# astaka-pe/SeMIGCN

Measured on AMD Instinct MI355X. Metric: GCN train iters/sec + edges-aggregated/sec, 1M-vert mesh, higher is better.
Workload: dtype bf16 storage / f32 accumulate; 1 GPU; SGCN train iteration (13 ChebConv K=3 + BN + LeakyReLU, fwd+loss+bwd, Adam every 5th) on a closed torus mesh 1000x1000: V=1000000 E=6000000 directed, grid vertex order, bf16 features; V=1000000, E=6000000, vertex_order=grid

## Files before the change

### include/semigcn.h

```cpp
#ifndef SEMIGCN_H
#define SEMIGCN_H

#include <stdint.h>

#ifdef __cplusplus
extern "C" {
#endif

#if defined(__GNUC__)
#define SG_API __attribute__((visibility("default")))
#else
#define SG_API
#endif

#define SG_ABI_VERSION 1

enum sg_status {
  SG_OK = 0,
  SG_ERR_INVALID = -1,
  SG_ERR_HIP = -2,
  SG_ERR_UNSUPPORTED = -3,
  SG_ERR_NO_DEVICE = -4
};

// ... 128 lines not shown
SG_API int sg_fill_emit(sg_fill* s, const float* vs, float* new_vs, int64_t* new_faces, uint8_t* filled_out, void* stream);

typedef struct sg_parts sg_parts;
SG_API int sg_parts_create(const int64_t* faces, int64_t F, int64_t V, int connectivity, void* stream, sg_parts** out);
SG_API int sg_parts_destroy(sg_parts* p);
SG_API int sg_parts_query(const sg_parts* p, int64_t* info);
SG_API int sg_parts_labels(const sg_parts* p, int64_t* face_label, int64_t* face_count, void* stream);
SG_API int sg_parts_select(sg_parts* p, const uint8_t* keep, void* stream, int64_t* n_vertices, int64_t* n_faces);
SG_API int sg_parts_emit(sg_parts* p, const float* vs, float* new_vs, int64_t* new_faces, int64_t* vertex_ids, int64_t* face_ids,
                         void* stream);

typedef struct sg_remesh sg_remesh;
SG_API int sg_remesh_create(const float* vs, int64_t V, const int64_t* faces, int64_t F, void* stream, sg_remesh** out);
SG_API int sg_remesh_destroy(sg_remesh* p);
SG_API int sg_remesh_query(const sg_remesh* p, int64_t* info);
SG_API int sg_remesh_split(sg_remesh* p, float thr2, int64_t max_rounds, void* stream, int64_t* counts, int64_t* n_rounds,
                           int64_t* n_long);
SG_API int sg_remesh_flip(sg_remesh* p, int64_t max_rounds, void* stream, int64_t* counts, int64_t* n_rounds, int64_t* deviation);
SG_API int sg_remesh_collapse(sg_remesh* p, float lo2, float thr2, int64_t max_rounds, void* stream, int64_t* counts,
                              int64_t* n_rounds, int64_t* n_short);
SG_API int sg_remesh_collapse_maps(const sg_remesh* p, int64_t* vertex_ids, int64_t* merged_into, void* stream);
SG_API int sg_remesh_export(const sg_remesh* p, float* vs, int64_t* faces, int64_t* parents, uint8_t* border, void* stream);
SG_API int sg_remesh_set_feature(sg_remesh* p, int enabled, double cos_t);
SG_API int sg_remesh_features(sg_remesh* p, void* stream, uint8_t* vclass, int64_t* crease_nbr, int64_t* n_crease);
SG_API int sg_remesh_crease_edges(const sg_remesh* p, int64_t* edges, void* stream);
SG_API int sg_crease_step(const float* in, float* out, const int64_t* crease_nbr, int64_t V, void* stream);

SG_API int sg_mesh_loss_finalize(const float* partial, int64_t nb, float n_v, float n_f, float w_pos, float k1, float* out,
                                 void* stream);
SG_API int64_t sg_mesh_loss_blocks(int64_t V, int64_t F);
SG_API int sg_mesh_loss_fwd(const float* pos, const int64_t* faces, const float* target_pos, const float* v_keep,
                            const float* target_fn, const float* f_keep, int64_t V, int64_t F, float* partial,
                            void* stream);
SG_API int sg_mesh_loss_bwd_det(const float* pos, const int64_t* faces, const float* target_pos, const float* v_keep,
                                const float* target_fn, const float* f_keep, const float* g, int64_t V, int64_t V_ext,
                                int64_t F, const sg_pool* incidence, float* corner_scratch, float* grad_pos, void* stream);
SG_API int sg_mesh_loss_bwd(const float* pos, const int64_t* faces, const float* target_pos, const float* v_keep,
                            const float* target_fn, const float* f_keep, const float* g, int64_t V, int64_t V_ext,
                            int64_t F, float* grad_pos, void* stream);

SG_API int64_t sg_bnf_blocks(int64_t F);
SG_API int64_t sg_bnf_scratch_bytes(int64_t F);
SG_API int sg_bnf_filter(const float* pos, const int64_t* faces, const int64_t* f2f, int64_t V, int64_t F, int loop,
                         float sigma_s, const float* start_fn, float* fn, float* n_filtered, float* loss_partial,
                         void* scratch, void* stream);
SG_API int sg_mesh_loss_cad_finalize(const float* partial, int64_t nb, float n_v, float n_f, float w_pos, float k1,
                                     const float* bnf_partial, int64_t nb_bnf, int64_t F, float k2, float* out, void* stream);
SG_API int sg_mesh_loss_cad_bwd_det(const float* pos, const int64_t* faces, const float* target_pos, const float* v_keep,
                                    const float* target_fn, const float* f_keep, const float* fn, const float* n_filtered,
                                    const float* g, int64_t V, int64_t V_ext, int64_t F, const sg_pool* incidence,
                                    float* corner_scratch, float* grad_pos, void* stream);

SG_API int sg_gemm_nt_takes_big_tile(int64_t M, int64_t N, int64_t K, int64_t lda, int64_t ldb, int64_t ldc);
SG_API int64_t sg_gemm_tile_rows(int64_t N);
SG_API int64_t sg_gemm_row_tiles(int64_t M, int64_t N);
SG_API int sg_gemm_nt(const void* A, int64_t lda, const void* B, int64_t ldb, const float* bias, void* C, int64_t ldc,
                      int64_t M, int64_t N, int64_t K, int dtype, float* moments, void* stream);
SG_API int64_t sg_gemm_tn_slabs(int64_t M, int64_t N, int64_t Kp);
SG_API int sg_gemm_tn_takes_big_tile(int64_t M, int64_t N, int64_t Kp, int64_t lda, int64_t ldb);
SG_API int sg_gemm_tn(const void* A, int64_t lda, const void* B, int64_t ldb, int64_t M, int64_t N, int64_t Kp, int dtype,
                      float* workspace, float* out, int64_t ldo, void* stream);
SG_API int sg_gemm_nt_f32_supported(int64_t M, int64_t N, int64_t K, int64_t lda, int64_t ldc);
SG_API int sg_gemm_nt_f32_pays(int64_t M, int64_t N, int64_t K);
SG_API int sg_gemm_nt_f32_variant(int64_t M);
SG_API int64_t sg_gemm_nt_f32_workspace(int64_t N, int64_t K);
SG_API int sg_gemm_nt_f32(const float* A, int64_t lda, const float* W, int64_t w_rs, int64_t w_cs, const float* bias, float* C,
                          int64_t ldc, int64_t M, int64_t N, int64_t K, void* workspace, int64_t workspace_bytes, void* stream);
SG_API int sg_gemm_tn_f32_supported(int64_t M, int64_t N, int64_t Kp, int64_t lda, int64_t ldb);
SG_API int64_t sg_gemm_tn_f32_workspace(int64_t M, int64_t N, int64_t Kp);
SG_API int sg_gemm_tn_f32(const float* A, int64_t lda, const float* B, int64_t ldb, int64_t M, int64_t N, int64_t Kp,
                          void* workspace, int64_t workspace_bytes, float* out, int64_t ldo, void* stream);
SG_API int sg_bn_stats_finalize_tiles(const float* partial, int64_t n_tiles, int64_t rows_per_tile, int64_t V, int64_t C,
                                      const float* gamma, const float* beta, float* running_mean, float* running_var,
                                      float momentum, float eps, float* out, int64_t* batches_tracked, void* stream);

SG_API int sg_input_bounds(const float* z1, int64_t V, float* partial_values, int64_t* partial_index, float* bounds, int64_t* arg,
                           void* stream);
SG_API int sg_input_prep_bwd_routed(const void* gX, int64_t ldg, const float* z1, const float* dm, const int64_t* rank,
                                    const float* bounds, const int64_t* arg, float* dz1, float* partial, float* d_bounds,
                                    int64_t V, int dtype, void* stream);
SG_API int64_t sg_input_prep_blocks(int64_t V);
SG_API int sg_input_prep(const float* z1, const float* dm, const int64_t* order, const float* lo, const float* hi, void* X,
                         int64_t ldx, int64_t V, int dtype, void* stream);
SG_API int sg_input_prep_bwd(const void* gX, int64_t ldg, const float* z1, const float* dm, const int64_t* rank,
                             const float* lo, const float* hi, float* dz1, float* partial, float* d_lo, float* d_hi, int64_t V,
                             int dtype, void* stream);

typedef struct sg_block {
  const sg_graph* graph;
  const sg_pool* pool;
  int32_t pool_mode;
  int32_t dtype;
  int32_t K;
  int32_t order;
  int32_t training;
  int32_t refresh_weights;
  int32_t need_dx;
  int32_t reserved_;
  int64_t V, V_out;
  int64_t Cin, Cout;
  float momentum, eps, slope;
  float reserved2_;
  const float* W[3];
  const float* bias;
  const float* gamma;
  const float* beta;
// ... 111 lines not shown
```

### semigcn_amd/capi.py

```python
from __future__ import annotations

import ctypes
import functools
from array import array as _array
import os
from ctypes import POINTER, byref, c_char_p, c_float, c_int, c_int32, c_int64, c_void_p
from typing import Optional

import torch

_LIB_NAME = "libsemigcn_hip.so"
_LIB_PATH = os.path.join(os.path.dirname(os.path.abspath(__file__)), _LIB_NAME)

SG_F32, SG_BF16 = 0, 1
_DTYPES = {torch.float32: SG_F32, torch.bfloat16: SG_BF16}


class SemigcnLibraryError(RuntimeError):
    """libsemigcn_hip.so is absent / unloadable, or a call into it failed."""


class sg_graph_info(ctypes.Structure):
    _fields_ = [("V_dst", c_int64), ("V_src", c_int64), ("nnz", c_int64),
                ("symmetric", c_int32), ("max_degree", c_int32)]
# ... 21 lines not shown


PHASE_CONV, PHASE_BN, PHASE_BWD_REDUCE, PHASE_BWD_A, PHASE_BWD_B = 1, 2, 4, 8, 16


class sg_part_step(ctypes.Structure):
    _fields_ = [("kind", c_int32), ("reserved_", c_int32), ("blocks", POINTER(sg_block)), ("n", c_int64),
                ("send", c_void_p), ("recv", c_void_p)]


STEP_BLOCKS, STEP_EXCHANGE, STEP_ALL_REDUCE, STEP_ALL_GATHER = 0, 1, 2, 3


class sg_trace_record(ctypes.Structure):
    _fields_ = [("kind", c_int32), ("dtype", c_int32), ("engine", c_int32), ("reserved_", c_int32),
                ("a", c_int64), ("b", c_int64), ("c", c_int64), ("ms", c_float), ("reserved2_", c_float)]


_SIGNATURES = {
    "sg_last_error": (c_char_p, []),
    "sg_abi_version": (c_int, []),
    "sg_device_count": (c_int, []),
    "sg_graph_create": (c_int, [c_void_p, c_int64, c_int64, c_void_p, POINTER(c_void_p)]),
    "sg_graph_create_rect": (c_int, [c_void_p, c_void_p, c_int64, c_int64, c_int64, c_void_p, c_void_p,
                                     POINTER(c_void_p)]),
    "sg_graph_create_rows": (c_int, [c_void_p, c_void_p, c_int64, c_int64, c_int64, c_void_p, c_void_p, c_void_p, c_void_p,
                                     POINTER(c_void_p)]),
    "sg_graph_destroy": (c_int, [c_void_p]),
    "sg_graph_query": (c_int, [c_void_p, POINTER(sg_graph_info)]),
    "sg_graph_is_reordered": (c_int, [c_void_p]),
    "sg_graph_export": (c_int, [c_void_p, c_void_p, c_void_p, c_void_p, c_void_p]),
    "sg_spmm": (c_int, [c_void_p, c_int, c_void_p, c_int64, c_void_p, c_int64, c_void_p, c_int64,
                        c_void_p, c_int64, c_int64, c_int, c_float, c_float, c_float, c_void_p]),
    "sg_graph_prepare": (c_int, [c_void_p, c_int64, c_int, c_void_p]),
    "sg_pool_create": (c_int, [c_void_p, c_void_p, c_int64, c_int64, c_int64, c_void_p, POINTER(c_void_p)]),
    "sg_pool_destroy": (c_int, [c_void_p]),
    "sg_pool_mean": (c_int, [c_void_p, c_void_p, c_int64, c_void_p, c_int64, c_int64, c_int, c_void_p]),
    "sg_pool_mean_bwd": (c_int, [c_void_p, c_void_p, c_int64, c_void_p, c_int64, c_int64, c_int, c_void_p]),
    "sg_unpool": (c_int, [c_void_p, c_void_p, c_int64, c_void_p, c_int64, c_int64, c_int, c_void_p]),
    "sg_unpool_bwd": (c_int, [c_void_p, c_void_p, c_int64, c_void_p, c_int64, c_int64, c_int, c_void_p]),
    "sg_tuning_set": (c_int, [c_int, c_int]),
    "sg_mesh_loss_blocks": (c_int64, [c_int64, c_int64]),
    "sg_mesh_loss_fwd": (c_int, [c_void_p] * 6 + [c_int64, c_int64, c_void_p, c_void_p]),
    "sg_mesh_loss_bwd": (c_int, [c_void_p] * 7 + [c_int64, c_int64, c_int64, c_void_p, c_void_p]),
    "sg_mesh_loss_bwd_det": (c_int, [c_void_p] * 7 + [c_int64, c_int64, c_int64, c_void_p, c_void_p, c_void_p, c_void_p]),
    "sg_col_blocks": (c_int64, [c_int64]),
    "sg_col_moments": (c_int, [c_void_p, c_int64, c_int64, c_int64, c_int, c_void_p, c_int64, c_void_p]),
    "sg_bn_merge": (c_int, [c_void_p, c_int64, c_int64, c_int64, c_void_p, c_void_p]),
    "sg_bn_stats_finalize": (c_int, [c_void_p, c_int64, c_int64, c_int64, c_void_p, c_void_p, c_void_p, c_void_p, c_float,
                                     c_float, c_void_p, c_void_p, c_void_p]),
    "sg_bn_stats_finalize_tiles": (c_int, [c_void_p, c_int64, c_int64, c_int64, c_int64, c_void_p, c_void_p, c_void_p,
                                           c_void_p, c_float, c_float, c_void_p, c_void_p, c_void_p]),
    "sg_gemm_nt_takes_big_tile": (c_int, [c_int64, c_int64, c_int64, c_int64, c_int64, c_int64]),
    "sg_gemm_tile_rows": (c_int64, [c_int64]),
    "sg_gemm_row_tiles": (c_int64, [c_int64, c_int64]),
    "sg_gemm_nt": (c_int, [c_void_p, c_int64, c_void_p, c_int64, c_void_p, c_void_p, c_int64, c_int64, c_int64, c_int64,
                           c_int, c_void_p, c_void_p]),
    "sg_gemm_nt_f32_supported": (c_int, [c_int64, c_int64, c_int64, c_int64, c_int64]),
    "sg_gemm_nt_f32_pays": (c_int, [c_int64, c_int64, c_int64]),
    "sg_gemm_nt_f32_variant": (c_int, [c_int64]),
    "sg_gemm_nt_f32_workspace": (c_int64, [c_int64, c_int64]),
    "sg_gemm_nt_f32": (c_int, [c_void_p, c_int64, c_void_p, c_int64, c_int64, c_void_p, c_void_p, c_int64, c_int64, c_int64,
                               c_int64, c_void_p, c_int64, c_void_p]),
    "sg_gemm_tn_f32_supported": (c_int, [c_int64, c_int64, c_int64, c_int64, c_int64]),
    "sg_gemm_tn_f32_workspace": (c_int64, [c_int64, c_int64, c_int64]),
    "sg_gemm_tn_f32": (c_int, [c_void_p, c_int64, c_void_p, c_int64, c_int64, c_int64, c_int64, c_void_p, c_int64, c_void_p,
                               c_int64, c_void_p]),
    "sg_gemm_tn_slabs": (c_int64, [c_int64, c_int64, c_int64]),
    "sg_gemm_tn_takes_big_tile": (c_int, [c_int64, c_int64, c_int64, c_int64, c_int64]),
    "sg_gemm_tn": (c_int, [c_void_p, c_int64, c_void_p, c_int64, c_int64, c_int64, c_int64, c_int, c_void_p, c_void_p, c_int64,
                           c_void_p]),
    "sg_thin_supported": (c_int, [c_int64, c_int64]),
    "sg_thin_tn_blocks": (c_int64, [c_int64]),
    "sg_thin_nt": (c_int, [c_void_p, c_int64, c_void_p, c_int64, c_void_p, c_void_p, c_int64, c_int64, c_int64, c_int64, c_int,
                           c_void_p]),
    "sg_thin_tn": (c_int, [c_void_p, c_int64, c_void_p, c_int64, c_int64, c_int64, c_int64, c_int, c_void_p, c_void_p, c_int64,
                           c_void_p]),
    "sg_bn_bwd_coeffs": (c_int, [c_void_p, c_int64, c_int64, ctypes.c_double, c_void_p, c_void_p, c_void_p, c_void_p,
                                 c_void_p, c_void_p, c_void_p]),
    "sg_bn_merge_tiles": (c_int, [c_void_p, c_int64, c_int64, c_int64, c_int64, c_void_p, c_void_p, c_void_p]),
    "sg_multi_add": (c_int, [c_int64, c_void_p, c_void_p, c_void_p, c_void_p, c_void_p, c_void_p]),
    "sg_input_bounds": (c_int, [c_void_p, c_int64, c_void_p, c_void_p, c_void_p, c_void_p, c_void_p]),
    "sg_input_prep_bwd_routed": (c_int, [c_void_p, c_int64, c_void_p, c_void_p, c_void_p, c_void_p, c_void_p, c_void_p, c_void_p,
                                         c_void_p, c_int64, c_int, c_void_p]),
    "sg_mesh_loss_finalize": (c_int, [c_void_p, c_int64, c_float, c_float, c_float, c_float, c_void_p, c_void_p]),
    "sg_bnf_blocks": (c_int64, [c_int64]),
    "sg_bnf_scratch_bytes": (c_int64, [c_int64]),
    "sg_bnf_filter": (c_int, [c_void_p, c_void_p, c_void_p, c_int64, c_int64, c_int, c_float] + [c_void_p] * 6),
    "sg_mesh_loss_cad_finalize": (c_int, [c_void_p, c_int64, c_float, c_float, c_float, c_float, c_void_p, c_int64, c_int64, c_float,
                                          c_void_p, c_void_p]),
    "sg_mesh_loss_cad_bwd_det": (c_int, [c_void_p] * 9 + [c_int64, c_int64, c_int64, c_void_p, c_void_p, c_void_p, c_void_p]),
    "sg_input_prep_blocks": (c_int64, [c_int64]),
    "sg_input_prep": (c_int, [c_void_p, c_void_p, c_void_p, c_void_p, c_void_p, c_void_p, c_int64, c_int64, c_int, c_void_p]),
    "sg_input_prep_bwd": (c_int, [c_void_p, c_int64, c_void_p, c_void_p, c_void_p, c_void_p, c_void_p, c_void_p, c_void_p,
                                  c_void_p, c_void_p, c_int64, c_int, c_void_p]),
    "sg_bn_finalize_ranks": (c_int, [c_void_p, c_int64, c_int64, c_void_p, c_void_p, c_void_p, c_void_p, c_float, c_float,
                                     c_void_p, c_void_p, c_void_p, c_void_p]),
    "sg_bn_finalize": (c_int, [c_void_p, ctypes.c_double, c_int64, c_void_p, c_void_p, c_void_p, c_void_p, c_float,
                               c_float, c_void_p, c_void_p]),
    "sg_scale_shift_act": (c_int, [c_void_p, c_int64, c_void_p, c_void_p, c_float, c_void_p, c_int64, c_int64,
                                   c_int64, c_int, c_void_p]),
    "sg_bn_act_bwd_reduce": (c_int, [c_void_p, c_int64, c_void_p, c_int64, c_void_p, c_void_p, c_void_p, c_void_p,
                                     c_float, c_void_p, c_int64, c_int64, c_int64, c_int, c_void_p]),
    "sg_bn_act_bwd_apply": (c_int, [c_void_p, c_int64, c_void_p, c_int64, c_void_p, c_void_p, c_void_p, c_void_p,
                                    c_void_p, c_void_p, c_void_p, c_float, c_void_p, c_int64, c_int64, c_int64, c_int,
                                    c_void_p]),
# ... 513 lines not shown


def bn_stats_finalize(partial: torch.Tensor, num_rows: int, gamma: torch.Tensor, beta: torch.Tensor,
                      running_mean: Optional[torch.Tensor], running_var: Optional[torch.Tensor], momentum: float,
                      eps: float, batches_tracked: Optional[torch.Tensor] = None) -> torch.Tensor:
    nb, _, C = partial.shape
    out = torch.empty((4, C), dtype=torch.float32, device=partial.device)
    for t, n in ((running_mean, "running_mean"), (running_var, "running_var")):
        if t is not None:
            _f32vec(t, C, n)
    with _on_device(partial.device):
        _check(load().sg_bn_stats_finalize(_ptr(partial), nb, int(num_rows), C, _ptr(_f32vec(gamma, C, "weight")),
                                           _ptr(_f32vec(beta, C, "bias")), _ptr(running_mean), _ptr(running_var),
                                           float(momentum), float(eps), _ptr(out), _counter(batches_tracked, partial),
                                           _stream(partial)), "sg_bn_stats_finalize")
    return out


def bn_stats_finalize_tiles(partial: torch.Tensor, rows_per_tile: int, num_rows: int, gamma: torch.Tensor,
                            beta: torch.Tensor, running_mean: Optional[torch.Tensor], running_var: Optional[torch.Tensor],
                            momentum: float, eps: float, batches_tracked: Optional[torch.Tensor] = None) -> torch.Tensor:
    nb, _, C = partial.shape
    out = torch.empty((4, C), dtype=torch.float32, device=partial.device)
    for t, n in ((running_mean, "running_mean"), (running_var, "running_var")):
        if t is not None:
            _f32vec(t, C, n)
    with _on_device(partial.device):
        _check(load().sg_bn_stats_finalize_tiles(_ptr(partial), nb, int(rows_per_tile), int(num_rows), C,
                                                 _ptr(_f32vec(gamma, C, "weight")), _ptr(_f32vec(beta, C, "bias")),
                                                 _ptr(running_mean), _ptr(running_var), float(momentum), float(eps),
                                                 _ptr(out), _counter(batches_tracked, partial), _stream(partial)),
               "sg_bn_stats_finalize_tiles")
    return out


def gemm_tile_rows(N: int) -> int:
    return _sizes("sg_gemm_tile_rows", int(N))


def gemm_nt_supported(A: torch.Tensor, B: torch.Tensor, ldc: int) -> bool:
    if A.dtype != torch.bfloat16 or B.dtype != torch.bfloat16 or not A.is_cuda or A.dim() != 2 or B.dim() != 2:
        return False
    if A.shape[1] != B.shape[1] or A.stride(1) != 1 or B.stride(1) != 1 or A.shape[0] == 0:
        return False
    K, N = A.shape[1], B.shape[0]
    return (K % 8 == 0 and N % 8 == 0 and A.stride(0) % 8 == 0 and B.stride(0) % 8 == 0 and ldc % 8 == 0
            and A.data_ptr() % 16 == 0 and B.data_ptr() % 16 == 0)


def gemm_nt_takes_big_tile(M: int, N: int, K: int, lda: int, ldb: int, ldc: int) -> bool:
    return bool(_sizes("sg_gemm_nt_takes_big_tile", int(M), int(N), int(K), int(lda), int(ldb), int(ldc)))


def gemm_nt(A: torch.Tensor, B: torch.Tensor, bias: Optional[torch.Tensor] = None, out: Optional[torch.Tensor] = None,
            moments: bool = False):
    _require_device(A, "A")
    _require_device(B, "B")
    M, K = A.shape
    N = B.shape[0]
    if out is None:
        out = torch.empty((M, N), dtype=torch.bfloat16, device=A.device)
    if out.shape != (M, N) or out.dtype != torch.bfloat16 or B.shape[1] != K:
        raise SemigcnLibraryError(f"gemm_nt shape mismatch: A {tuple(A.shape)} B {tuple(B.shape)} out {tuple(out.shape)}")
    if bias is not None:
        _f32vec(bias, N, "bias")
    mom = None
    if moments:
        mom = torch.empty((_sizes("sg_gemm_row_tiles", M, N), 2, N), dtype=torch.float32, device=A.device)
    with _on_device(A.device):
        _check(load().sg_gemm_nt(_ptr(A), _rows2d(A, "A"), _ptr(B), _rows2d(B, "B"), _ptr(bias), _ptr(out),
                                 _rows2d(out, "out"), M, N, K, SG_BF16, _ptr(mom), _stream(A)), "sg_gemm_nt")
    return (out, mom) if moments else out


THIN_ELEMS = 256


def thin_shape(N: int, K: int) -> bool:
    return bool(_sizes("sg_thin_supported", int(N), int(K)))


def thin_supported(A: torch.Tensor, N: int, K: int) -> bool:
    return (A.is_cuda and A.dim() == 2 and A.stride(1) == 1 and A.dtype in (torch.float32, torch.bfloat16)
            and N >= 1 and K >= 1 and thin_shape(N, K) and A.shape[0] > 0)


def thin_nt(X: torch.Tensor, W: torch.Tensor, bias: Optional[torch.Tensor] = None, out: Optional[torch.Tensor] = None) -> torch.Tensor:
    _require_device(X, "X")
    V, K = X.shape
    N = W.shape[0]
    W = W if (W.dtype == torch.float32 and W.stride(1) == 1) else W.float().contiguous()
    if out is None:
        out = torch.empty((V, N), dtype=X.dtype, device=X.device)
    if out.shape != (V, N) or out.dtype != X.dtype or W.shape[1] != K or out.stride(1) != 1 or X.stride(1) != 1:
        raise SemigcnLibraryError(f"thin_nt shape mismatch: X {tuple(X.shape)} W {tuple(W.shape)} out {tuple(out.shape)}")
    if bias is not None:
        _f32vec(bias, N, "bias")
    with _on_device(X.device):
        _check(load().sg_thin_nt(_ptr(X), _rows2d(X, "X"), _ptr(W), _rows2d(W, "W"), _ptr(bias), _ptr(out), _rows2d(out, "out"),
                                 V, N, K, dtype_code(X), _stream(X)), "sg_thin_nt")
    return out


def thin_tn(A: torch.Tensor, B: torch.Tensor) -> torch.Tensor:
    _require_device(A, "A")
    _require_device(B, "B")
# ... 1036 lines not shown
```

### semigcn_amd/csrc/api.hip

```cpp
#include <stdarg.h>

#include <new>

#include <mutex>

#include "sg_common.h"

namespace sg {

static thread_local std::string t_error;

void set_error(const char* fmt, ...) {
  char buf[1024];
  va_list ap;
  va_start(ap, fmt);
  vsnprintf(buf, sizeof(buf), fmt, ap);
  va_end(ap);
  t_error = buf;
}

namespace {

struct ScopedFree {
  void* p = nullptr;
// ... 698 lines not shown
    rc = run_csr(incidence->by_coarse, nullptr, nullptr, corner_scratch, 3, nullptr, 0, nullptr, 0, grad_pos, 3, 3, SG_F32,
                 1.f, 0.f, 0.f, stream);
    if (rc != SG_OK) return rc;
  }
  return launch_mesh_loss_bwd_vertex_add(pos, target_pos, v_keep, g, V, grad_pos, stream);
}

SG_API int64_t sg_col_blocks(int64_t V) { return col_blocks(V); }

SG_API int sg_col_moments(const void* X, int64_t ldx, int64_t V, int64_t C, int dtype, float* partial, int64_t nb,
                          void* stream) {
  SG_REQUIRE(V >= 0 && C >= 0, "sg_col_moments: negative size");
  if (V == 0 || C == 0) return SG_OK;
  SG_REQUIRE(X && partial && ldx >= C, "sg_col_moments: bad argument");
  return launch_col_reduce(0, X, ldx, nullptr, 0, nullptr, nullptr, nullptr, nullptr, 0.f, partial, nb, V, C, dtype,
                           (hipStream_t)stream);
}

SG_API int sg_bn_merge(const float* partial, int64_t nb, int64_t V, int64_t C, float* stats, void* stream) {
  SG_REQUIRE(V > 0 && C >= 0 && partial && stats, "sg_bn_merge: bad argument");
  return launch_bn_merge(partial, nb, V, C, stats, (hipStream_t)stream);
}

SG_API int sg_bn_merge_tiles(const float* partial, int64_t n_tiles, int64_t rows_per_tile, int64_t V, int64_t C, float* stats,
                             float* count_out, void* stream) {
  SG_REQUIRE(V > 0 && C >= 0 && partial && stats, "sg_bn_merge_tiles: bad argument");
  return launch_bn_merge_tiles(partial, n_tiles, rows_per_tile, V, C, stats, count_out, (hipStream_t)stream);
}

SG_API int sg_bn_stats_finalize(const float* partial, int64_t nb, int64_t V, int64_t C, const float* gamma,
                                const float* beta, float* running_mean, float* running_var, float momentum, float eps,
                                float* out, int64_t* batches_tracked, void* stream) {
  SG_REQUIRE(V > 1 && C >= 0 && partial && gamma && beta && out, "sg_bn_stats_finalize: bad argument");
  SG_REQUIRE((running_mean == nullptr) == (running_var == nullptr),
             "sg_bn_stats_finalize: give both running buffers or none");
  return launch_bn_stats_finalize(partial, nb, V, C, gamma, beta, running_mean, running_var, momentum, eps, out,
                                  batches_tracked, (hipStream_t)stream);
}

SG_API int sg_bn_stats_finalize_tiles(const float* partial, int64_t n_tiles, int64_t rows_per_tile, int64_t V, int64_t C,
                                      const float* gamma, const float* beta, float* running_mean, float* running_var,
                                      float momentum, float eps, float* out, int64_t* batches_tracked, void* stream) {
  SG_REQUIRE(V > 1 && C >= 0 && partial && gamma && beta && out, "sg_bn_stats_finalize_tiles: bad argument");
  SG_REQUIRE((running_mean == nullptr) == (running_var == nullptr),
             "sg_bn_stats_finalize_tiles: give both running buffers or none");
  return launch_bn_stats_finalize_tiles(partial, n_tiles, rows_per_tile, V, C, gamma, beta, running_mean, running_var,
                                        momentum, eps, out, batches_tracked, (hipStream_t)stream);
}

SG_API int sg_gemm_nt_takes_big_tile(int64_t M, int64_t N, int64_t K, int64_t lda, int64_t ldb, int64_t ldc) {
  return gemm_nt_takes_big_tile(M, N, K, lda, ldb, ldc) ? 1 : 0;
}

SG_API int64_t sg_gemm_tile_rows(int64_t N) { return gemm_tile_rows(N); }

SG_API int64_t sg_gemm_row_tiles(int64_t M, int64_t N) {
  const int64_t r = gemm_tile_rows(N);
  return M <= 0 ? 0 : (M + r - 1) / r;
}

SG_API int sg_gemm_nt(const void* A, int64_t lda, const void* B, int64_t ldb, const float* bias, void* C, int64_t ldc,
                      int64_t M, int64_t N, int64_t K, int dtype, float* moments, void* stream) {
  SG_REQUIRE(M >= 0 && N >= 0 && K >= 0, "sg_gemm_nt: negative size");
  if (M == 0 || N == 0) return SG_OK;
  SG_REQUIRE(A && B && C && K > 0, "sg_gemm_nt: null operand or K = 0");
  SG_REQUIRE(lda >= K && ldb >= K && ldc >= N, "sg_gemm_nt: row stride shorter than the row");
  return launch_gemm_nt(A, lda, B, ldb, bias, C, ldc, M, N, K, dtype, moments, (hipStream_t)stream);
}

SG_API int64_t sg_gemm_tn_slabs(int64_t M, int64_t N, int64_t Kp) { return gemm_tn_slabs(M, N, Kp); }

SG_API int sg_gemm_tn_takes_big_tile(int64_t M, int64_t N, int64_t Kp, int64_t lda, int64_t ldb) {
  return gemm_tn_takes_big_tile(M, N, Kp, lda, ldb) ? 1 : 0;
}

SG_API int sg_gemm_tn(const void* A, int64_t lda, const void* B, int64_t ldb, int64_t M, int64_t N, int64_t Kp, int dtype,
                      float* workspace, float* out, int64_t ldo, void* stream) {
  SG_REQUIRE(M >= 0 && N >= 0 && Kp >= 0, "sg_gemm_tn: negative size");
  if (N == 0 || Kp == 0) return SG_OK;
  SG_REQUIRE(out != nullptr && ldo >= Kp, "sg_gemm_tn: bad output");
  if (M == 0) {
    SG_HIP_TRY(hipMemset2DAsync(out, ldo * sizeof(float), 0, Kp * sizeof(float), N, (hipStream_t)stream));
    return SG_OK;
  }
  SG_REQUIRE(A && B && workspace && lda >= N && ldb >= Kp, "sg_gemm_tn: null operand or short row stride");
  return launch_gemm_tn(A, lda, B, ldb, M, N, Kp, dtype, workspace, out, ldo, (hipStream_t)stream);
}

SG_API int sg_gemm_nt_f32_supported(int64_t M, int64_t N, int64_t K, int64_t lda, int64_t ldc) {
  return (gemm_nt_f32s_supported(M, N, K, lda, ldc) || (M >= 0 && mid_shape(N, K) && lda % 4 == 0 && ldc % 4 == 0)) ? 1 : 0;
}

SG_API int sg_gemm_nt_f32_variant(int64_t M) { return gemm_nt_f32s_variant(M); }

SG_API int sg_gemm_nt_f32_pays(int64_t M, int64_t N, int64_t K) {
  return (mid_shape(N, K) || split_nt_pays(M, N, K)) ? 1 : 0;
}

SG_API int64_t sg_gemm_nt_f32_workspace(int64_t N, int64_t K) {
  return (N > 0 && K > 0 && !mid_shape(N, K)) ? gemm_nt_f32s_workspace(N, K) : 0;
}

SG_API int sg_gemm_nt_f32(const float* A, int64_t lda, const float* W, int64_t w_rs, int64_t w_cs, const float* bias, float* C,
                          int64_t ldc, int64_t M, int64_t N, int64_t K, void* workspace, int64_t workspace_bytes, void* stream) {
  SG_REQUIRE(M >= 0 && N >= 0 && K >= 0, "sg_gemm_nt_f32: negative size");
  if (M == 0 || N == 0) return SG_OK;
// ... 238 lines not shown
```

### semigcn_amd/csrc/gemm_mfma.hip

```cpp
#include "sg_common.h"

namespace sg {
namespace {

typedef __attribute__((ext_vector_type(8))) __bf16 bf16x8;
typedef __attribute__((ext_vector_type(4))) float f32x4;
typedef uint32_t u32x4 __attribute__((ext_vector_type(4)));

constexpr int kThreads = 256;
constexpr int kBK = 64;
constexpr int kRowBytes = 128;

struct GemmArgs {
  const uint16_t* A; int64_t lda;
  const uint16_t* B; int64_t ldb;
  const float* bias;
  uint16_t* C; int64_t ldc;
  float* moments;
  int M, N, K;
  int n_col_tiles, n_tiles;
  int a_plog; int64_t a_pstride;
  int c_plog; int64_t c_pstride;
};

// ... 186 lines not shown

  constexpr int CPR = BN / 8;
#pragma unroll
  for (int i = 0; i < BM * CPR / kThreads; ++i) {
    const int q = tid + kThreads * i;
    const int r = q / CPR, c = q % CPR;
    const int gc = col0 + c * 8;
    if (r < rows_valid && gc < g.N)
      *(u32x4*)(g.C + (int64_t)(row0 + r) * g.ldc + plane_off(gc, g.c_plog, g.c_pstride)) = *(const u32x4*)(ldsC + r * C_PITCH + c * 16);
  }

  if (MOMENTS && tid < BN && col0 + tid < g.N) {
    const float* red = (const float*)(lds + LDS_BYTES - RED_BYTES);
    float n = red[WAVES_M * BN * 2], mean = red[tid * 2], m2 = red[tid * 2 + 1];
#pragma unroll
    for (int w = 1; w < WAVES_M; ++w) {
      const float nb = red[WAVES_M * BN * 2 + w], mb = red[(w * BN + tid) * 2], qb = red[(w * BN + tid) * 2 + 1];
      const float tot = n + nb;
      const float wgt = tot > 0.f ? nb / tot : 0.f;
      const float d = mb - mean;
      mean = fmaf(d, wgt, mean);
      m2 += qb + d * d * n * wgt;
      n = tot;
    }
    float* out = g.moments + (int64_t)(tile / g.n_col_tiles) * 2 * g.N;
    out[col0 + tid] = mean;
    out[g.N + col0 + tid] = m2;
  }
}

template <int WAVES_M, int WAVES_N, int MT, int NT>
int launch(GemmArgs g, hipStream_t stream) {
  constexpr int BM = WAVES_M * MT * 16, BN = WAVES_N * NT * 16;
  g.n_col_tiles = (g.N + BN - 1) / BN;
  const int64_t tiles = (int64_t)((g.M + BM - 1) / BM) * g.n_col_tiles;
  SG_REQUIRE(tiles <= INT32_MAX, "sg_gemm_nt: too many tiles");
  g.n_tiles = (int)tiles;
  if (g.moments) gemm_nt_bf16<WAVES_M, WAVES_N, MT, NT, true><<<g.n_tiles, kThreads, 0, stream>>>(g);
  else gemm_nt_bf16<WAVES_M, WAVES_N, MT, NT, false><<<g.n_tiles, kThreads, 0, stream>>>(g);
  SG_HIP_TRY(hipGetLastError());
  return SG_OK;
}

inline bool a16(const void* p) { return ((uintptr_t)p & 15) == 0; }

int g_gemm_tile = 0;

constexpr int64_t kBigMinWeightElems = 90000;
constexpr int64_t kBigMinRows = 16384;

bool wide_tile(int64_t N) { return g_gemm_tile == 2 && N > 64; }
bool tile_192(int64_t N) { return g_gemm_tile != 1 && g_gemm_tile != 4 && (N == 192 || (g_gemm_tile == 5 && N == 384)); }

}

int gemm_tile_rows(int64_t N) { return wide_tile(N) ? 64 : 128; }

bool gemm_nt_takes_big_tile(int64_t M, int64_t N, int64_t K, int64_t lda, int64_t ldb, int64_t ldc) {
  if (g_gemm_tile == 1 || g_gemm_tile == 2 || !gemm_nt_256_supported(M, N, K, lda, ldb, ldc)) return false;
  return g_gemm_tile == 3 || (K * N > kBigMinWeightElems && M >= kBigMinRows);
}

int set_gemm_tuning(int value) {
  g_gemm_tile = value;
  return SG_OK;
}

int launch_gemm_nt(const void* A, int64_t lda, const void* B, int64_t ldb, const float* bias, void* C, int64_t ldc,
                   int64_t M, int64_t N, int64_t K, int dtype, float* moments, hipStream_t stream, Planes pa, Planes pc) {
  if (dtype != SG_BF16) {
    set_error("sg_gemm_nt: bf16 operands only (dtype %d); fp32 products stay with the BLAS library", dtype);
    return SG_ERR_UNSUPPORTED;
  }
  if (K % 8 || N % 8 || lda % 8 || ldb % 8 || ldc % 8 || !a16(A) || !a16(B) || !a16(C)) {
    set_error("sg_gemm_nt: needs K, N and the row strides to be multiples of 8 and 16-byte aligned operands "
              "(K=%lld N=%lld lda=%lld ldb=%lld ldc=%lld)", (long long)K, (long long)N, (long long)lda, (long long)ldb,
              (long long)ldc);
    return SG_ERR_UNSUPPORTED;
  }
  SG_REQUIRE(M <= INT32_MAX && N <= INT32_MAX && K <= INT32_MAX, "sg_gemm_nt: size out of range");
  const bool planes = pa.on() || pc.on();
  if (planes) {
    SG_REQUIRE((!pa.on() || (pa.log2 >= 3 && pa.log2 < 31 && pa.stride % 8 == 0)) &&
               (!pc.on() || (pc.log2 >= 3 && pc.log2 < 31 && pc.stride % 8 == 0)),
               "sg_gemm_nt: planes need >= 8 columns each and a plane stride that is a multiple of 8 elements");
    SG_REQUIRE(!wide_tile(N), "sg_gemm_nt: operands kept as planes run on the 128-row tiles only");
  }
  if (!planes && moments == nullptr && gemm_nt_takes_big_tile(M, N, K, lda, ldb, ldc))
    return launch_gemm_nt_256(A, lda, B, ldb, bias, C, ldc, M, N, K, stream);
  GemmArgs g;
  g.a_plog = pa.log2; g.a_pstride = pa.stride;
  g.c_plog = pc.log2; g.c_pstride = pc.stride;
  g.A = (const uint16_t*)A; g.lda = lda;
  g.B = (const uint16_t*)B; g.ldb = ldb;
  g.bias = bias;
  g.C = (uint16_t*)C; g.ldc = ldc;
  g.moments = moments;
  g.M = (int)M; g.N = (int)N; g.K = (int)K;
  g.n_col_tiles = g.n_tiles = 0;
  if (wide_tile(N)) return launch<1, 4, 4, 4>(g, stream);
  if (tile_192(N) && !moments) return launch<2, 2, 4, 6>(g, stream);
  if (N > 64) return launch<2, 2, 4, 4>(g, stream);
  if (N > 32) return launch<4, 1, 2, 4>(g, stream);
  if (N > 16) return launch<4, 1, 2, 2>(g, stream);
  return launch<4, 1, 2, 1>(g, stream);
}

namespace {

typedef __attribute__((ext_vector_type(4))) __bf16 bf16x4;
constexpr int kTnStep = 64;
constexpr int kTnMaxSlabRows = 8192;

__host__ __device__ inline int tn_slab_rows(int64_t M, int64_t n_tiles) {
  int64_t rows = (M * n_tiles / 512 + kTnStep - 1) / kTnStep * kTnStep;
  rows = rows < 512 ? 512 : rows;
  return (int)(rows > kTnMaxSlabRows ? kTnMaxSlabRows : rows);
}

struct TnArgs {
  const uint16_t* A; int64_t lda;
  const uint16_t* B; int64_t ldb;
  float* W;
  int M, N, Kp;
  int tiles_n, tiles_k, n_tiles, n_blocks, slab_rows;
  int a_plog; int64_t a_pstride;
  int b_plog; int64_t b_pstride;
};

__device__ __forceinline__ int tn_swz(int row) { return (row & 3) | (((row >> 3) & 1) << 2); }

__global__ __launch_bounds__(kThreads, 3) void gemm_tn_bf16(const TnArgs g) {
  constexpr int TILE_BYTES = kTnStep * 256;
  __shared__ __attribute__((aligned(16))) uint8_t lds[2 * TILE_BYTES];
  uint8_t* const ldsA = lds;
  uint8_t* const ldsB = lds + TILE_BYTES;
  const int tid = threadIdx.x, lane = tid & 63, wave = tid >> 6;
  const int wn = wave >> 1, wk = wave & 1;
  const int blk = xcd_run(blockIdx.x, g.n_blocks);
  const int slab = blk / g.n_tiles, tile = blk % g.n_tiles;
// ... 211 lines not shown
```

### semigcn_amd/csrc/sg_common.h

```cpp
#pragma once
#include <hip/hip_runtime.h>
#include <stdint.h>
#include <stdio.h>
#include <atomic>
#include <string>

#include "semigcn.h"

namespace sg {

void set_error(const char* fmt, ...);

#define SG_HIP_TRY(expr)                                                              \
  do {                                                                                \
    hipError_t e__ = (expr);                                                          \
    if (e__ != hipSuccess) {                                                          \
      sg::set_error("%s failed: %s (%s:%d)", #expr, hipGetErrorString(e__), __FILE__, \
                    __LINE__);                                                        \
      return SG_ERR_HIP;                                                              \
    }                                                                                 \
  } while (0)

#define SG_REQUIRE(cond, ...)      \
  do {                             \
// ... 156 lines not shown
                       int64_t ldy, int64_t C, int dtype, hipStream_t stream);

int64_t col_blocks(int64_t V);
int launch_col_reduce(int mode, const void* A, int64_t lda, const void* H, int64_t ldh, const float* scale,
                      const float* shift, const float* mean, const float* invstd, float slope, float* out,
                      int64_t nblk, int64_t V, int64_t C, int dtype, hipStream_t stream);
int launch_bn_merge(const float* partial, int64_t nb, int64_t V, int64_t C, float* stats, hipStream_t stream);
int launch_bn_stats_finalize(const float* partial, int64_t nb, int64_t V, int64_t C, const float* gamma,
                             const float* beta, float* running_mean, float* running_var, float momentum, float eps,
                             float* out, int64_t* batches_tracked, hipStream_t stream);
int launch_bn_bwd_coeffs(const float* partial, int64_t nb, int64_t C, double N, const float* gamma,
                         const float* invstd, float* out, float* acc_dweight, float* acc_dbias, const float* count_dev,
                         hipStream_t stream);
int launch_bn_merge_tiles(const float* partial, int64_t nb, int64_t rpb, int64_t V, int64_t C, float* stats,
                          float* count_out, hipStream_t stream);
int launch_bn_finalize_ranks(const float* all, int64_t world, int64_t C, const float* gamma, const float* beta,
                             float* running_mean, float* running_var, float momentum, float eps, float* out,
                             float* out_n, int64_t* batches_tracked, hipStream_t stream);
int launch_bn_finalize(const float* stats, double N, int64_t C, const float* gamma, const float* beta,
                       float* running_mean, float* running_var, float momentum, float eps, float* out,
                       hipStream_t stream);
int launch_col_apply(int mode, const void* A, int64_t lda, const void* H, int64_t ldh, const float* scale,
                     const float* shift, const float* mean, const float* invstd, const float* kk, const float* c1,
                     const float* c2, float slope, void* Y, int64_t ldy, int64_t V, int64_t C, int dtype,
                     hipStream_t stream, float* colsum = nullptr);
int64_t col_apply_blocks(int64_t V, int64_t C, int dtype);
int launch_colsum_finalize(const float* partial, int64_t nb, int64_t C, float* out, hipStream_t stream, float* acc = nullptr);

int launch_bn_stats_finalize_tiles(const float* partial, int64_t nb, int64_t rpb, int64_t V, int64_t C, const float* gamma,
                                   const float* beta, float* running_mean, float* running_var, float momentum, float eps,
                                   float* out, int64_t* batches_tracked, hipStream_t stream);
constexpr int kMultiAddMax = 8;
int launch_multi_add(int n, const float* const* srcs, const int64_t* src_ld, const int64_t* rows, const int64_t* cols,
                     float* const* dsts, hipStream_t stream);

int64_t input_prep_blocks(int64_t V);
int launch_input_prep(const float* z1, const float* dm, const int64_t* order, const float* lo, const float* hi, void* X,
                      int64_t ldx, int64_t V, int dtype, hipStream_t stream);
int launch_input_prep_bwd(const void* gX, int64_t ldg, const float* z1, const float* dm, const int64_t* rank, const float* lo,
                          const float* hi, float* dz1, float* partial, float* d_lo, float* d_hi, int64_t V, int dtype,
                          hipStream_t stream);

int launch_input_bounds(const float* z1, int64_t V, float* pv, int64_t* pi, float* bounds, int64_t* arg, hipStream_t stream);
int launch_bounds_route(const float* d_lo, const float* d_hi, const int64_t* arg, float* dz1, hipStream_t stream);
int launch_mesh_loss_finalize(const float* partial, int64_t nb, float n_v, float n_f, float w_pos, float k1, float* out,
                              hipStream_t stream);

int gemm_tile_rows(int64_t N);
int set_gemm_tuning(int value);
int launch_gemm_nt(const void* A, int64_t lda, const void* B, int64_t ldb, const float* bias, void* C, int64_t ldc,
                   int64_t M, int64_t N, int64_t K, int dtype, float* moments, hipStream_t stream, Planes pa = {}, Planes pc = {});

bool gemm_nt_takes_big_tile(int64_t M, int64_t N, int64_t K, int64_t lda, int64_t ldb, int64_t ldc);
bool gemm_nt_256_supported(int64_t M, int64_t N, int64_t K, int64_t lda, int64_t ldb, int64_t ldc);
int launch_gemm_nt_256(const void* A, int64_t lda, const void* B, int64_t ldb, const float* bias, void* C, int64_t ldc,
                       int64_t M, int64_t N, int64_t K, hipStream_t stream);
bool gemm_tn_256_supported(int64_t M, int64_t N, int64_t Kp, int64_t lda, int64_t ldb);
int gemm_tn_256_slabs(int64_t M, int64_t N, int64_t Kp);
int launch_gemm_tn_256(const void* A, int64_t lda, const void* B, int64_t ldb, int64_t M, int64_t N, int64_t Kp,
                       float* workspace, hipStream_t stream);
bool gemm_tn_takes_big_tile(int64_t M, int64_t N, int64_t Kp, int64_t lda, int64_t ldb);
int64_t gemm_tn_slabs(int64_t M, int64_t N, int64_t Kp);
int launch_gemm_tn(const void* A, int64_t lda, const void* B, int64_t ldb, int64_t M, int64_t N, int64_t Kp, int dtype,
                   float* workspace, float* out, int64_t ldo, hipStream_t stream, const GradSink* sink = nullptr, Planes pa = {},
                   Planes pb = {});

bool gemm_nt_f32s_supported(int64_t M, int64_t N, int64_t K, int64_t lda, int64_t ldc);
int64_t gemm_nt_f32s_workspace(int64_t N, int64_t K);
int launch_gemm_nt_f32s(const float* A, int64_t lda, const float* W, int64_t w_rs, int64_t w_cs, const float* bias, float* C,
                        int64_t ldc, int64_t M, int64_t N, int64_t K, void* ws, int64_t ws_bytes, hipStream_t stream,
                        const void* prepacked = nullptr, int64_t variant_rows = 0);
int gemm_nt_f32s_variant(int64_t M);
int launch_pack_split(const float* W, int64_t w_rs, int64_t w_cs, int64_t variant_rows, int64_t N, int64_t K, void* out,
                      hipStream_t stream);
int set_split_tuning(int value);
int set_bn_rows_tuning(int value);
bool split_engine_enabled(int kind = 0);
bool gemm_tn_f32s_supported(int64_t M, int64_t N, int64_t Kp, int64_t lda, int64_t ldb);
int64_t gemm_tn_f32s_workspace(int64_t M, int64_t N, int64_t Kp);
int launch_split_tn_reduce(const float* ws, int n_slabs, int64_t N, int64_t Kp, float* out, int64_t ldo, const GradSink* sink,
                           hipStream_t stream);
constexpr int64_t kSplitNtPaysRows = 16384;
bool split_nt_pays(int64_t M, int64_t N, int64_t K);
bool mid_shape(int64_t N, int64_t K);
int64_t mid_tn_workspace(int64_t M, int64_t N, int64_t Kp);
int launch_mid_nt(const float* X, int64_t ldx, const float* W, int64_t w_rs, int64_t w_cs, const float* bias, float* Y, int64_t ldy,
                  int64_t M, int64_t N, int64_t K, hipStream_t stream);
int launch_mid_tn(const float* A, int64_t lda, const float* B, int64_t ldb, int64_t M, int64_t N, int64_t Kp, float* ws, float* out,
                  int64_t ldo, hipStream_t stream, const GradSink* sink);
int launch_gemm_tn_f32s(const float* A, int64_t lda, const float* B, int64_t ldb, int64_t M, int64_t N, int64_t Kp, void* ws,
                        int64_t ws_bytes, float* out, int64_t ldo, hipStream_t stream, const GradSink* sink = nullptr);

int64_t mesh_loss_blocks(int64_t V, int64_t F);
int launch_mesh_loss_fwd(const float* pos, const int64_t* faces, const float* tpos, const float* vkeep, const float* tfn,
                         const float* fkeep, int64_t V, int64_t F, float* partial, hipStream_t stream);
int launch_mesh_loss_bwd(const float* pos, const int64_t* faces, const float* tpos, const float* vkeep, const float* tfn,
                         const float* fkeep, const float* g, int64_t V, int64_t V_ext, int64_t F, float* grad,
                         hipStream_t stream);

int mesh_edges(const int64_t* faces, int64_t F, int64_t V, int64_t* edges_out, int64_t* f2f_out,
               int64_t* n_edges_out, int* manifold_out, hipStream_t stream);
int launch_mask_dilate(const Csr& c, const uint64_t* in, uint64_t* out, int64_t W, hipStream_t stream);
int launch_face_mask(const int64_t* faces, int64_t F, int64_t V, const uint64_t* vbits, uint64_t* fbits, int64_t W,
                     hipStream_t stream);
int surface_create(const float* vs, int64_t V, const int64_t* faces, int64_t F, hipStream_t stream, sg_surface** out);
void destroy_surface(sg_surface* s);
// ... 105 lines not shown
```

Baseline: 38.64 iter/s.

## Add persistent row-tile MFMA GEMM holding A rows in registers across column tiles

Adds a persistent bf16 NT GEMM kernel where each workgroup keeps a 128-row slab of A (whole K) in registers and streams B column tiles through swizzled LDS, with double-buffered prefetch of the next B tile and next A slab. It is dispatched by default for the specific (N,K) ChebConv shapes (e.g. 384x256, 192x128) when M is large and no moments or input planes are required. The intent is to read A once instead of once per column tile and so cut global traffic on the wide-output GEMMs. The cost is high register pressure, since whole-K A fragments stay resident, and a shape whitelist that may not match every layer.

Result: no change. 38.93 iter/s (median of 6 runs) (+0.8%).

```diff
diff --git a/include/semigcn.h b/include/semigcn.h
--- a/include/semigcn.h
+++ b/include/semigcn.h
@@ -204,6 +204,7 @@
                                     float* corner_scratch, float* grad_pos, void* stream);
 
 SG_API int sg_gemm_nt_takes_big_tile(int64_t M, int64_t N, int64_t K, int64_t lda, int64_t ldb, int64_t ldc);
+SG_API int sg_gemm_nt_takes_row_tile(int64_t M, int64_t N, int64_t K, int64_t lda, int64_t ldb, int64_t ldc);
 SG_API int64_t sg_gemm_tile_rows(int64_t N);
 SG_API int64_t sg_gemm_row_tiles(int64_t M, int64_t N);
 SG_API int sg_gemm_nt(const void* A, int64_t lda, const void* B, int64_t ldb, const float* bias, void* C, int64_t ldc,
diff --git a/semigcn_amd/capi.py b/semigcn_amd/capi.py
--- a/semigcn_amd/capi.py
+++ b/semigcn_amd/capi.py
@@ -97,6 +97,7 @@
     "sg_bn_stats_finalize_tiles": (c_int, [c_void_p, c_int64, c_int64, c_int64, c_int64, c_void_p, c_void_p, c_void_p,
                                            c_void_p, c_float, c_float, c_void_p, c_void_p, c_void_p]),
     "sg_gemm_nt_takes_big_tile": (c_int, [c_int64, c_int64, c_int64, c_int64, c_int64, c_int64]),
+    "sg_gemm_nt_takes_row_tile": (c_int, [c_int64, c_int64, c_int64, c_int64, c_int64, c_int64]),
     "sg_gemm_tile_rows": (c_int64, [c_int64]),
     "sg_gemm_row_tiles": (c_int64, [c_int64, c_int64]),
     "sg_gemm_nt": (c_int, [c_void_p, c_int64, c_void_p, c_int64, c_void_p, c_void_p, c_int64, c_int64, c_int64, c_int64,
@@ -716,6 +717,10 @@
     return bool(_sizes("sg_gemm_nt_takes_big_tile", int(M), int(N), int(K), int(lda), int(ldb), int(ldc)))
 
 
+def gemm_nt_takes_row_tile(M: int, N: int, K: int, lda: int, ldb: int, ldc: int) -> bool:
+    return bool(_sizes("sg_gemm_nt_takes_row_tile", int(M), int(N), int(K), int(lda), int(ldb), int(ldc)))
+
+
 def gemm_nt(A: torch.Tensor, B: torch.Tensor, bias: Optional[torch.Tensor] = None, out: Optional[torch.Tensor] = None,
             moments: bool = False):
     _require_device(A, "A")
diff --git a/semigcn_amd/csrc/api.hip b/semigcn_amd/csrc/api.hip
--- a/semigcn_amd/csrc/api.hip
+++ b/semigcn_amd/csrc/api.hip
@@ -774,6 +774,10 @@
   return gemm_nt_takes_big_tile(M, N, K, lda, ldb, ldc) ? 1 : 0;
 }
 
+SG_API int sg_gemm_nt_takes_row_tile(int64_t M, int64_t N, int64_t K, int64_t lda, int64_t ldb, int64_t ldc) {
+  return gemm_nt_takes_row_tile(M, N, K, lda, ldb, ldc) ? 1 : 0;
+}
+
 SG_API int64_t sg_gemm_tile_rows(int64_t N) { return gemm_tile_rows(N); }
 
 SG_API int64_t sg_gemm_row_tiles(int64_t M, int64_t N) {
diff --git a/semigcn_amd/csrc/gemm_mfma.hip b/semigcn_amd/csrc/gemm_mfma.hip
--- a/semigcn_amd/csrc/gemm_mfma.hip
+++ b/semigcn_amd/csrc/gemm_mfma.hip
@@ -262,6 +262,8 @@
 bool wide_tile(int64_t N) { return g_gemm_tile == 2 && N > 64; }
 bool tile_192(int64_t N) { return g_gemm_tile != 1 && g_gemm_tile != 4 && (N == 192 || (g_gemm_tile == 5 && N == 384)); }
 
+constexpr int64_t kRowTileWins[][2] = {{384, 256}, {192, 128}, {96, 64}, {48, 32}};
+
 }
 
 int gemm_tile_rows(int64_t N) { return wide_tile(N) ? 64 : 128; }
@@ -269,6 +271,15 @@
 bool gemm_nt_takes_big_tile(int64_t M, int64_t N, int64_t K, int64_t lda, int64_t ldb, int64_t ldc) {
   if (g_gemm_tile == 1 || g_gemm_tile == 2 || !gemm_nt_256_supported(M, N, K, lda, ldb, ldc)) return false;
   return g_gemm_tile == 3 || (K * N > kBigMinWeightElems && M >= kBigMinRows);
+}
+
+bool gemm_nt_takes_row_tile(int64_t M, int64_t N, int64_t K, int64_t lda, int64_t ldb, int64_t ldc) {
+  if ((g_gemm_tile != 0 && g_gemm_tile != 6) || !gemm_nt_rowtile_supported(M, N, K, lda, ldb, ldc)) return false;
+  if (g_gemm_tile == 6) return true;
+  if (M < kBigMinRows) return false;
+  for (const auto& w : kRowTileWins)
+    if (N == w[0] && K == w[1]) return true;
+  return false;
 }
 
 int set_gemm_tuning(int value) {
@@ -296,6 +307,8 @@
                "sg_gemm_nt: planes need >= 8 columns each and a plane stride that is a multiple of 8 elements");
     SG_REQUIRE(!wide_tile(N), "sg_gemm_nt: operands kept as planes run on the 128-row tiles only");
   }
+  if (!pa.on() && moments == nullptr && gemm_nt_takes_row_tile(M, N, K, lda, ldb, ldc))
+    return launch_gemm_nt_rowtile(A, lda, B, ldb, bias, C, ldc, M, N, K, stream, pc);
   if (!planes && moments == nullptr && gemm_nt_takes_big_tile(M, N, K, lda, ldb, ldc))
     return launch_gemm_nt_256(A, lda, B, ldb, bias, C, ldc, M, N, K, stream);
   GemmArgs g;
diff --git a/semigcn_amd/csrc/gemm_rowtile.hip b/semigcn_amd/csrc/gemm_rowtile.hip
--- /dev/null
+++ b/semigcn_amd/csrc/gemm_rowtile.hip
@@ -0,0 +1,222 @@
+#include "sg_common.h"
+
+namespace sg {
+namespace {
+
+typedef __attribute__((ext_vector_type(8))) __bf16 bf16x8;
+typedef __attribute__((ext_vector_type(4))) float f32x4;
+typedef float f32x2 __attribute__((ext_vector_type(2)));
+typedef __bf16 bf16x2 __attribute__((ext_vector_type(2)));
+typedef uint32_t u32x4 __attribute__((ext_vector_type(4)));
+
+constexpr int kRtThreads = 256;
+constexpr int kRtBM = 128;
+constexpr int kRtBN = 64;
+constexpr int kRtMaxN = 1024;
+constexpr int kRtPlane = 128;
+
+struct RowTileArgs {
+  const uint16_t* A; int64_t lda;
+  const uint16_t* B; int64_t ldb;
+  const float* bias;
+  uint16_t* C; int64_t ldc;
+  int M, N;
+  int n_col_tiles, n_row_tiles;
+  int c_plog; int64_t c_pstride;
+};
+
+__device__ __forceinline__ int rt_xcd_run(int b, int nblocks) {
+  const int q = nblocks >> 3, r = nblocks & 7;
+  const int xcd = b & 7, slot = b >> 3;
+  return (xcd < r ? xcd * (q + 1) : r * (q + 1) + (xcd - r) * q) + slot;
+}
+
+template <int K, int WGS>
+__global__ __launch_bounds__(kRtThreads, WGS) void gemm_nt_rowtile(const RowTileArgs g) {
+  static_assert(K == 32 || K == 64 || K == 128 || K == 256, "K is held whole in registers");
+  constexpr int P = (K + 63) / 64;
+  constexpr int NKS = K / 32;
+  constexpr int B_PLANE = kRtBN * kRtPlane;
+  constexpr int A_STAGE = 32 * kRtPlane;
+  __shared__ __attribute__((aligned(16))) uint8_t ldsB[P * B_PLANE];
+  __shared__ __attribute__((aligned(16))) uint8_t ldsA[4 * A_STAGE];
+  __shared__ __attribute__((aligned(16))) float ldsBias[kRtMaxN + kRtBN];
+
+  const int tid = threadIdx.x, lane = tid & 63, wave = tid >> 6;
+  const int fr = lane & 15, fq = lane >> 4;
+  const int nblocks = (int)gridDim.x;
+  int tile = rt_xcd_run((int)blockIdx.x, nblocks);
+  if (tile >= g.n_row_tiles) return;
+
+  for (int c = tid; c < g.n_col_tiles * kRtBN; c += kRtThreads) ldsBias[c] = (g.bias != nullptr && c < g.N) ? g.bias[c] : 0.f;
+
+  const int s_c = tid & 7;
+  int s_k[P];
+#pragma unroll
+  for (int p = 0; p < P; ++p) {
+    const int k = p * 64 + s_c * 8;
+    s_k[p] = k < K ? k : 0;
+  }
+  u32x4 rb[P][2];
+  int b_dst[2];
+#pragma unroll
+  for (int h = 0; h < 2; ++h) {
+    const int r = (tid >> 3) + 32 * h;
+    b_dst[h] = r * kRtPlane + ((s_c ^ (r & 7)) << 4);
+  }
+  auto fetch_b = [&](int ct) {
+#pragma unroll
+    for (int h = 0; h < 2; ++h) {
+      int n = ct * kRtBN + (tid >> 3) + 32 * h;
+      n = n < g.N ? n : g.N - 1;
+      const uint16_t* src = g.B + (int64_t)n * g.ldb;
+#pragma unroll
+      for (int p = 0; p < P; ++p) rb[p][h] = *(const u32x4*)(src + s_k[p]);
+    }
+  };
+  auto stash_b = [&]() {
+#pragma unroll
+    for (int p = 0; p < P; ++p)
+#pragma unroll
+      for (int h = 0; h < 2; ++h) *(u32x4*)(ldsB + p * B_PLANE + b_dst[h]) = rb[p][h];
+  };
+  u32x4 ra[P][4];
+  uint8_t* const stage = ldsA + wave * A_STAGE;
+  int a_dst[4];
+#pragma unroll
+  for (int h = 0; h < 4; ++h) {
+    const int r = (lane >> 3) + 8 * h;
+    a_dst[h] = r * kRtPlane + ((s_c ^ (r & 7)) << 4);
+  }
+  auto fetch_a = [&](int t) {
+#pragma unroll
+    for (int h = 0; h < 4; ++h) {
+      int m = t * kRtBM + wave * 32 + (lane >> 3) + 8 * h;
+      m = m < g.M ? m : g.M - 1;
+      const uint16_t* src = g.A + (int64_t)m * g.lda;
+#pragma unroll
+      for (int p = 0; p < P; ++p) ra[p][h] = *(const u32x4*)(src + s_k[p]);
+    }
+  };
+  int f_off[2];
+#pragma unroll
+  for (int ks = 0; ks < 2; ++ks) f_off[ks] = fr * kRtPlane + ((((ks << 2) | fq) ^ (fr & 7)) << 4);
+  bf16x8 af[2][NKS];
+  auto stage_a = [&]() {
+#pragma unroll
+    for (int p = 0; p < P; ++p) {
+#pragma unroll
+      for (int h = 0; h < 4; ++h) *(u32x4*)(stage + a_dst[h]) = ra[p][h];
+      __builtin_amdgcn_wave_barrier();
+#pragma unroll
+      for (int mi = 0; mi < 2; ++mi)
+#pragma unroll
+        for (int ks = 0; ks < 2; ++ks)
+          if (2 * p + ks < NKS) af[mi][2 * p + ks] = *(const bf16x8*)(stage + mi * 16 * kRtPlane + f_off[ks]);
+      __builtin_amdgcn_wave_barrier();
+    }
+  };
+
+  fetch_b(0);
+  fetch_a(tile);
+  stash_b();
+  stage_a();
+  __syncthreads();
+
+  f32x4 acc[2][4];
+#pragma unroll
+  for (int mi = 0; mi < 2; ++mi)
+#pragma unroll
+    for (int j = 0; j < 4; ++j) acc[mi][j] = f32x4{0.f, 0.f, 0.f, 0.f};
+
+  const int nc = g.n_col_tiles;
+  for (;;) {
+    const int next = tile + nblocks;
+    const bool more = next < g.n_row_tiles;
+    const int row0 = tile * kRtBM + wave * 32;
+    for (int ct = 0; ct < nc; ++ct) {
+      fetch_b(ct + 1 < nc ? ct + 1 : 0);
+      if (ct == 0 && more) fetch_a(next);
+#pragma unroll
+      for (int s = 0; s < NKS; ++s) {
+        bf16x8 bfr[4];
+#pragma unroll
+        for (int j = 0; j < 4; ++j) bfr[j] = *(const bf16x8*)(ldsB + (s >> 1) * B_PLANE + j * 16 * kRtPlane + f_off[s & 1]);
+#pragma unroll
+        for (int mi = 0; mi < 2; ++mi)
+#pragma unroll
+          for (int j = 0; j < 4; ++j)
+            acc[mi][j] = __builtin_amdgcn_mfma_f32_16x16x32_bf16(bfr[j], af[mi][s], acc[mi][j], 0, 0, 0);
+      }
+      __syncthreads();
+      stash_b();
+      const int col0 = ct * kRtBN;
+#pragma unroll
+      for (int mi = 0; mi < 2; ++mi) {
+        const int row = row0 + mi * 16 + fr;
+#pragma unroll
+        for (int jp = 0; jp < 2; ++jp) {
+          uint32_t lo[2], hi[2];
+#pragma unroll
+          for (int jj = 0; jj < 2; ++jj) {
+            const int j = 2 * jp + jj;
+            const f32x4 bv = *(const f32x4*)(ldsBias + col0 + j * 16 + fq * 4);
+            const f32x4 v = acc[mi][j] + bv;
+            lo[jj] = __builtin_bit_cast(uint32_t, __builtin_convertvector(f32x2{v[0], v[1]}, bf16x2));
+            hi[jj] = __builtin_bit_cast(uint32_t, __builtin_convertvector(f32x2{v[2], v[3]}, bf16x2));
+            acc[mi][j] = f32x4{0.f, 0.f, 0.f, 0.f};
+          }
+          const auto sa = __builtin_amdgcn_permlane16_swap(lo[0], lo[1], false, false);
+          const auto sb = __builtin_amdgcn_permlane16_swap(hi[0], hi[1], false, false);
+          const int gc = col0 + jp * 32 + (fq & 1) * 16 + (fq >> 1) * 8;
+          if (row < g.M && gc < g.N)
+            *(u32x4*)(g.C + (int64_t)row * g.ldc + plane_off(gc, g.c_plog, g.c_pstride)) = u32x4{sa[0], sb[0], sa[1], sb[1]};
+        }
+      }
+      __syncthreads();
+    }
+    if (!more) break;
+    stage_a();
+    tile = next;
+  }
+}
+
+template <int K, int WGS>
+int launch_rowtile(RowTileArgs g, int cus, hipStream_t stream) {
+  const int want = WGS * cus;
+  const int grid = g.n_row_tiles < want ? g.n_row_tiles : want;
+  gemm_nt_rowtile<K, WGS><<<grid, kRtThreads, 0, stream>>>(g);
+  SG_HIP_TRY(hipGetLastError());
+  return SG_OK;
+}
+
+}
+
+bool gemm_nt_rowtile_supported(int64_t M, int64_t N, int64_t K, int64_t lda, int64_t ldb, int64_t ldc) {
+  return (K == 32 || K == 64 || K == 128 || K == 256) && N > K && N <= kRtMaxN && N % 8 == 0 && M >= 1 &&
+         (M + kRtBM - 1) / kRtBM <= INT32_MAX / kRtBM && lda % 8 == 0 && ldb % 8 == 0 && ldc % 8 == 0;
+}
+
+int launch_gemm_nt_rowtile(const void* A, int64_t lda, const void* B, int64_t ldb, const float* bias, void* C, int64_t ldc,
+                           int64_t M, int64_t N, int64_t K, hipStream_t stream, Planes pc) {
+  SG_REQUIRE(gemm_nt_rowtile_supported(M, N, K, lda, ldb, ldc), "sg_gemm_nt (row-tile kernel): unsupported shape");
+  SG_REQUIRE((((uintptr_t)A | (uintptr_t)B | (uintptr_t)C) & 15) == 0, "sg_gemm_nt (row-tile kernel): misaligned operand");
+  RowTileArgs g;
+  g.A = (const uint16_t*)A; g.lda = lda;
+  g.B = (const uint16_t*)B; g.ldb = ldb;
+  g.bias = bias;
+  g.C = (uint16_t*)C; g.ldc = ldc;
+  g.M = (int)M; g.N = (int)N;
+  g.n_col_tiles = (int)((N + kRtBN - 1) / kRtBN);
+  g.n_row_tiles = (int)((M + kRtBM - 1) / kRtBM);
+  g.c_plog = pc.log2; g.c_pstride = pc.stride;
+  int dev = 0, cus = 256;
+  SG_HIP_TRY(hipGetDevice(&dev));
+  SG_HIP_TRY(hipDeviceGetAttribute(&cus, hipDeviceAttributeMultiprocessorCount, dev));
+  if (K == 256) return launch_rowtile<256, 2>(g, cus, stream);
+  if (K == 128) return launch_rowtile<128, 2>(g, cus, stream);
+  if (K == 64) return launch_rowtile<64, 3>(g, cus, stream);
+  return launch_rowtile<32, 3>(g, cus, stream);
+}
+
+}
diff --git a/semigcn_amd/csrc/sg_common.h b/semigcn_amd/csrc/sg_common.h
--- a/semigcn_amd/csrc/sg_common.h
+++ b/semigcn_amd/csrc/sg_common.h
@@ -232,6 +232,10 @@
                    int64_t M, int64_t N, int64_t K, int dtype, float* moments, hipStream_t stream, Planes pa = {}, Planes pc = {});
 
 bool gemm_nt_takes_big_tile(int64_t M, int64_t N, int64_t K, int64_t lda, int64_t ldb, int64_t ldc);
+bool gemm_nt_takes_row_tile(int64_t M, int64_t N, int64_t K, int64_t lda, int64_t ldb, int64_t ldc);
+bool gemm_nt_rowtile_supported(int64_t M, int64_t N, int64_t K, int64_t lda, int64_t ldb, int64_t ldc);
+int launch_gemm_nt_rowtile(const void* A, int64_t lda, const void* B, int64_t ldb, const float* bias, void* C, int64_t ldc,
+                           int64_t M, int64_t N, int64_t K, hipStream_t stream, Planes pc = {});
 bool gemm_nt_256_supported(int64_t M, int64_t N, int64_t K, int64_t lda, int64_t ldb, int64_t ldc);
 int launch_gemm_nt_256(const void* A, int64_t lda, const void* B, int64_t ldb, const float* bias, void* C, int64_t ldc,
                        int64_t M, int64_t N, int64_t K, hipStream_t stream);
```
